# google/dynibar

Hardware: AMD Instinct MI355X
Metric: rays/sec (64 samples x 8 src views) (higher is better)
Workload: dtype f32 in / f32 accumulate; products from two half-float parts per operand (22-bit operands, 3 of the 4 partial products on the f16 matrix pipe, ~2^-20 relative per product); the exact 6-term bf16 build is tested beside it

## Files before the change

dynibar_amd/build.py:

```python
from __future__ import annotations

import os
import subprocess
import sys

HERE = os.path.dirname(os.path.abspath(__file__))
CSRC = os.path.join(HERE, 'csrc')
OUT = os.path.join(CSRC, 'libdynibar_hip.so')
OUT_X6 = os.path.join(CSRC, 'libdynibar_hip_x6.so')
OUT_X1 = os.path.join(CSRC, 'libdynibar_hip_x1.so')
UNITS = [
    ('dyn_geometry.hip', ['-ffp-contract=off', '-munsafe-fp-atomics']),
    ('dyn_nets.hip', []),
    ('dyn_encoder.hip', ['-munsafe-fp-atomics']),
    ('dyn_train.hip', ['-munsafe-fp-atomics']),
    ('dyn_comm.hip', []),
]
COMMON = ['--offload-arch=gfx950', '-O3', '-std=c++17', '-fPIC', '-Wall', '-Wno-unused-function']
FLAVOURS = [
    ('dyn_nets_x6.o', OUT_X6, ['-DDYN_SPLIT_TERMS=6', '-DDYN_SPLIT_F16=0']),
    ('dyn_nets_x1.o', OUT_X1, ['-DDYN_SPLIT_TERMS=1']),
]


def _deps():
  return [os.path.join(CSRC, f) for f in os.listdir(CSRC) if f.endswith(('.hip', '.h'))] + [
      os.path.join(os.path.dirname(HERE), 'include', 'dynibar_hip.h')]


STAMP = os.path.join(CSRC, '.build_stamp')


def _stamp():
  import hashlib
  h = hashlib.sha256(repr((COMMON, UNITS, [(o, os.path.basename(out), f) for o, out, f in FLAVOURS])).encode())
  for d in sorted(_deps() + [os.path.abspath(__file__)]):
    h.update(os.path.basename(d).encode())
    with open(d, 'rb') as f:
      h.update(f.read())
  return h.hexdigest()


def build(force=False, verbose=True):
  hipcc = os.environ.get('HIPCC', '/opt/rocm/bin/hipcc')
  units = [(s, f) for s, f in UNITS if os.path.exists(os.path.join(CSRC, s))]
  stamp = _stamp()
  if not force and all(os.path.exists(p) for p in [OUT, STAMP] + [out for _, out, _ in FLAVOURS]) and open(STAMP).read().strip() == stamp:
    return OUT
  if os.path.exists(STAMP):
    os.remove(STAMP)
  from concurrent.futures import ThreadPoolExecutor
  jobs = []
  for src, flags in units:
    obj = os.path.join(CSRC, src.replace('.hip', '.o'))
    jobs.append((obj, [hipcc] + COMMON + flags + ['-c', os.path.join(CSRC, src), '-o', obj]))
  for obj, _, flags in FLAVOURS:
    jobs.append((os.path.join(CSRC, obj), [hipcc] + COMMON + flags + ['-c', os.path.join(CSRC, 'dyn_nets.hip'), '-o', os.path.join(CSRC, obj)]))

  def run(job):
    if verbose:
      print(' '.join(job[1]), flush=True)
    subprocess.check_call(job[1])
    return job[0]

  with ThreadPoolExecutor(max_workers=int(os.environ.get('DYNIBAR_BUILD_JOBS', '6'))) as ex:
    built = list(ex.map(run, jobs))
  objs = built[:len(units)]
  cmd = [hipcc, '--offload-arch=gfx950', '-shared', '-fPIC'] + objs + ['-ldl', '-o', OUT]
  if verbose:
    print(' '.join(cmd), flush=True)
  subprocess.check_call(cmd)
  for flavour, (_, out, _) in zip(built[len(units):], FLAVOURS):
    subprocess.check_call([hipcc, '--offload-arch=gfx950', '-shared', '-fPIC', objs[0], flavour] + objs[2:] + ['-ldl', '-o', out])
  if _stamp() == stamp:
    with open(STAMP, 'w') as f:
      f.write(stamp + '\n')
  return OUT


if __name__ == '__main__':
  print(build(force='--force' in sys.argv))
```

dynibar_amd/csrc/dyn_mlp.h:

```cpp
#pragma once
#include <utility>

#include "dyn_device.h"

#ifndef DYN_EXCLUSIVE_CU
#define DYN_EXCLUSIVE_CU 1
#endif
#if DYN_EXCLUSIVE_CU && defined(__AMDGCN__)
#define DYN_CLAIM_REGISTER_FILE() asm volatile("; the whole register file" ::: "v255", "a255")
#else
#define DYN_CLAIM_REGISTER_FILE()
#endif
#define DYN_NET_THREADS 256
#define DYN_VIEW_THREADS 512

__host__ __device__ constexpr int dyn_fi(int r, int h) { return (r & 3) + 8 * (r >> 2) + 4 * h; }

__device__ __forceinline__ f32x16 mfma32(float a, float b, f32x16 c) { return __builtin_amdgcn_mfma_f32_32x32x2f32(a, b, c, 0, 0, 0); }

template <int NT>
__device__ __forceinline__ void acc_zero(f32x16 (&acc)[NT]) {
#pragma unroll
  for (int t = 0; t < NT; ++t)
#pragma unroll
// ... 105 lines not shown
  a = seg_sum<VSEG>(a, 0, 0); b = seg_sum<VSEG>(b, 0, 0); c = seg_sum<VSEG>(c, 0, 0); d = seg_sum<VSEG>(d, 0, 0);
}
template <int VSEG>
__device__ __forceinline__ float seg_min(float v, int, int) {
  return seg_reduce<VSEG>(v, [](float a, float b) { return fminf(a, b); });
}
template <int VSEG>
__device__ __forceinline__ float seg_max(float v, int, int) {
  return seg_reduce<VSEG>(v, [](float a, float b) { return fmaxf(a, b); });
}

template <int NTI>
__device__ __forceinline__ float row_dot(const f32x16 (&act)[NTI], const float* tab) {
  const int h = (threadIdx.x & 63) >> 5;
  const float4* t4 = reinterpret_cast<const float4*>(tab + h * 16 * NTI);
  float s = 0.f;
#pragma unroll
  for (int t = 0; t < NTI; ++t)
#pragma unroll
    for (int q = 0; q < 4; ++q) {
      const float4 w = t4[t * 4 + q];
      s = fmaf(act[t][q * 4 + 0], w.x, s);
      s = fmaf(act[t][q * 4 + 1], w.y, s);
      s = fmaf(act[t][q * 4 + 2], w.z, s);
      s = fmaf(act[t][q * 4 + 3], w.w, s);
    }
  return s + __shfl_xor(s, 32);
}

#ifndef DYN_SPLIT_TERMS
#define DYN_SPLIT_TERMS 3
#endif
#ifndef DYN_SPLIT_F16
#define DYN_SPLIT_F16 1
#endif
#if DYN_SPLIT_F16 && DYN_SPLIT_TERMS == 6
#error "the half-float engine has one or two parts per operand (DYN_SPLIT_TERMS == 1 or 3)"
#endif
#if !DYN_SPLIT_F16 && DYN_SPLIT_TERMS == 1
#error "the one-product engine multiplies IEEE halves (DYN_SPLIT_F16 == 1)"
#endif
#if DYN_SPLIT_TERMS == 1
#define DYN_SPLIT_PARTS 1
#define B6_CHUNK_PAIRS 48
#elif DYN_SPLIT_TERMS == 3
#define DYN_SPLIT_PARTS 2
#define B6_CHUNK_PAIRS 24
#elif DYN_SPLIT_TERMS == 6
#define DYN_SPLIT_PARTS 3
#define B6_CHUNK_PAIRS 16
#else
#error "DYN_SPLIT_TERMS must be 1, 3 or 6"
#endif
#define DYN_BIAS_ONE(h) ((DYN_SPLIT_TERMS == 1 || (h) == 0) ? 1.0f : 0.0f)
typedef __bf16 bf16x8 __attribute__((ext_vector_type(8)));
typedef __bf16 bf16x2v __attribute__((ext_vector_type(2)));
typedef _Float16 f16x8 __attribute__((ext_vector_type(8)));
typedef _Float16 f16x2v __attribute__((ext_vector_type(2)));
typedef float f32x2v __attribute__((ext_vector_type(2)));
typedef unsigned u32x4v __attribute__((ext_vector_type(4)));

#define B6_PAIR_FLOATS (DYN_SPLIT_PARTS * 256)
#define B6_CHUNK (B6_CHUNK_PAIRS * B6_PAIR_FLOATS)

#ifdef DYN_PHASE_TIMING
__device__ unsigned long long g_phase[3][2][160];
#define DYN_PHASE_ON (threadIdx.x == 0 && (blockIdx.x == 0 || blockIdx.x == gridDim.x / 2))
#define DYN_PHASE(i)                                                                                  \
  do {                                                                                                \
    if (DYN_PHASE_ON) g_phase[PHASE_KID][blockIdx.x != 0][i] = __builtin_readcyclecounter();          \
  } while (0)
extern "C" int dyn_debug_phases(unsigned long long* out) {
  return hipMemcpyFromSymbol(out, HIP_SYMBOL(g_phase), sizeof(g_phase)) == hipSuccess ? 0 : 1;
}
#define DYN_PHASE_T0 const unsigned long long phase_t0 = __builtin_readcyclecounter();
#ifdef DYN_PHASE_SKEW
__device__ unsigned long long g_skew[8][4];
extern "C" int dyn_debug_skew(unsigned long long* out) { return hipMemcpyFromSymbol(out, HIP_SYMBOL(g_skew), sizeof(g_skew)) == hipSuccess ? 0 : 1; }
extern "C" int dyn_debug_skew_reset(void) { unsigned long long z[32] = {0}; return hipMemcpyToSymbol(HIP_SYMBOL(g_skew), z, sizeof(z)) == hipSuccess ? 0 : 1; }
#endif
#define DYN_PHASE_WAIT(R, c)                                                                          \
  do {                                                                                                \
    if (DYN_PHASE_ON && (c) < 64) {                                                                   \
      g_phase[(R).kid][blockIdx.x != 0][32 + (c)] = __builtin_readcyclecounter() - phase_t0;          \
      g_phase[(R).kid][blockIdx.x != 0][96 + (c)] = phase_t0;                                         \
    }                                                                                                 \
  } while (0)
#define DYN_PHASE_RING_KID(R, k) (R).kid = (k)
#else
#define DYN_PHASE(i)
#define DYN_PHASE_T0
#define DYN_PHASE_WAIT(R, c)
#define DYN_PHASE_RING_KID(R, k)
#endif

struct WeightRing6 {
  const float* gbase;
  float* buf;
  int next, total;
  int skip_at, skip_n;
  int round;
  int half;
  unsigned lds_wave;
  unsigned lane_off;
  int fill, issued;
  int nbuf;
// ... 192 lines not shown
#if DYN_SPLIT_PARTS == 3
  f32x2v mf = {__uint_as_float(mid << 16), __uint_as_float(mid & 0xffff0000u)};
  f32x2v r2 = r1 - mf;
  lo = __builtin_bit_cast(unsigned, __builtin_convertvector(r2, bf16x2v));
#else
  lo = 0u;
#endif
#endif
}

__device__ __forceinline__ f32x16 mfma_bf16(u32x4v a, u32x4v b, f32x16 c) {
#if DYN_SPLIT_F16
  return __builtin_amdgcn_mfma_f32_32x32x16_f16(__builtin_bit_cast(f16x8, a), __builtin_bit_cast(f16x8, b), c, 0, 0, 0);
#else
  return __builtin_amdgcn_mfma_f32_32x32x16_bf16(__builtin_bit_cast(bf16x8, a), __builtin_bit_cast(bf16x8, b), c, 0, 0, 0);
#endif
}

__host__ __device__ constexpr int b6_layer_chunks(int NT, int NSLOTS, int CP = B6_CHUNK_PAIRS) {
  return (((NSLOTS + 7) / 8) + (CP / NT) - 1) / (CP / NT);
}

struct B6A {
  u32x4v hi, mid, lo;
};
__device__ __forceinline__ B6A b6_load_a(const float* pair, int lane) {
  const u32x4v* w = reinterpret_cast<const u32x4v*>(pair) + lane;
  B6A a;
  a.hi = w[0];
#if DYN_SPLIT_PARTS >= 2
  a.mid = w[64];
#endif
#if DYN_SPLIT_PARTS == 3
  a.lo = w[128];
#endif
  return a;
}

template <int NSLOTS, int P0, int P1, class Feed>
__device__ __forceinline__ void b6_split_pairs(Feed& feed, int g, u32x4v& bh, u32x4v& bm, u32x4v& bl) {
#pragma unroll
  for (int p2 = P0; p2 < P1; ++p2) {
    const float v0 = (g * 8 + 2 * p2 < NSLOTS) ? feed(g * 8 + 2 * p2) : 0.f;
    const float v1 = (g * 8 + 2 * p2 + 1 < NSLOTS) ? feed(g * 8 + 2 * p2 + 1) : 0.f;
    unsigned h_, m_, l_;
    split3_pair(v0, v1, h_, m_, l_);
    bh[p2] = h_; bm[p2] = m_; bl[p2] = l_;
  }
}

#ifndef B6_AHEAD
#define B6_AHEAD 1
#endif
template <int NT, int NSLOTS, int AHEAD = B6_AHEAD, class Feed>
__device__ __forceinline__ void mlp_layer_b6(WeightRing6& R, f32x16 (&acc)[NT], Feed&& feed) {
  constexpr int NG = (NSLOTS + 7) / 8;
  constexpr int GPC = B6_CHUNK_PAIRS / NT;
  constexpr int NCH = (NG + GPC - 1) / GPC;
  static_assert(B6_CHUNK_PAIRS % NT == 0, "tiles per layer must divide the pairs of a chunk");
  static_assert(NT == 1 || NT == 2 || NT == 4 || NT == 8, "output tiles per layer");
  const int lane = threadIdx.x & 63;
  u32x4v bh, bm, bl, nh, nm, nl;
  b6_split_pairs<NSLOTS, 0, 4>(feed, 0, bh, bm, bl);
  nh = bh; nm = bm; nl = bl;
  __builtin_amdgcn_sched_barrier(0);
#pragma unroll
  for (int c = 0; c < NCH; ++c) {
    const float* buf = ring6_acquire(R);
    constexpr int NPC_MAX = B6_CHUNK_PAIRS;
    const int npc = (NG - c * GPC < GPC ? NG - c * GPC : GPC) * NT;
    B6A q[AHEAD + 1];
#pragma unroll
    for (int i = 0; i < AHEAD; ++i)
      if (i < npc) q[i] = b6_load_a(buf + i * B6_PAIR_FLOATS, lane);
    __builtin_amdgcn_sched_barrier(0);
#pragma unroll
    for (int pr = 0; pr < NPC_MAX; ++pr) {
      if (pr < npc) {
        const int gi = pr / NT, t = pr % NT;
        const int g = c * GPC + gi;
        ring6_feed(R, pr, npc);
#if B6_PRIO_FLIP && (B6_PRIO_MODE == 1 || B6_PRIO_MODE == 5)
        if (pr % B6_PRIO_FLIP == 0) ring6_prio_flip(R, (pr / B6_PRIO_FLIP) & 1);
#endif
        if (pr + AHEAD < npc) q[(pr + AHEAD) % (AHEAD + 1)] = b6_load_a(buf + (pr + AHEAD) * B6_PAIR_FLOATS, lane);
        if (g + 1 < NG) {
          if (NT == 1) b6_split_pairs<NSLOTS, 0, 4>(feed, g + 1, nh, nm, nl);
          if (NT == 2 && t == 0) b6_split_pairs<NSLOTS, 0, 2>(feed, g + 1, nh, nm, nl);
          if (NT == 2 && t == 1) b6_split_pairs<NSLOTS, 2, 4>(feed, g + 1, nh, nm, nl);
          if (NT == 4 && t == 0) b6_split_pairs<NSLOTS, 0, 1>(feed, g + 1, nh, nm, nl);
          if (NT == 4 && t == 1) b6_split_pairs<NSLOTS, 1, 2>(feed, g + 1, nh, nm, nl);
          if (NT == 4 && t == 2) b6_split_pairs<NSLOTS, 2, 3>(feed, g + 1, nh, nm, nl);
          if (NT == 4 && t == 3) b6_split_pairs<NSLOTS, 3, 4>(feed, g + 1, nh, nm, nl);
          if (NT == 8 && t == 0) b6_split_pairs<NSLOTS, 0, 1>(feed, g + 1, nh, nm, nl);
          if (NT == 8 && t == 2) b6_split_pairs<NSLOTS, 1, 2>(feed, g + 1, nh, nm, nl);
          if (NT == 8 && t == 4) b6_split_pairs<NSLOTS, 2, 3>(feed, g + 1, nh, nm, nl);
          if (NT == 8 && t == 6) b6_split_pairs<NSLOTS, 3, 4>(feed, g + 1, nh, nm, nl);
        }
        const B6A& cur = q[pr % (AHEAD + 1)];
#if DYN_SPLIT_TERMS == 6
        acc[t] = mfma_bf16(cur.lo, bh, acc[t]);
        acc[t] = mfma_bf16(cur.hi, bl, acc[t]);
        acc[t] = mfma_bf16(cur.mid, bm, acc[t]);
#endif
#if DYN_SPLIT_TERMS != 1
        acc[t] = mfma_bf16(cur.mid, bh, acc[t]);
        acc[t] = mfma_bf16(cur.hi, bm, acc[t]);
#endif
        acc[t] = mfma_bf16(cur.hi, bh, acc[t]);
        if (t == NT - 1) { bh = nh; bm = nm; bl = nl; }
        __builtin_amdgcn_sched_barrier(0);
      }
    }
  }
}

#ifndef B6D_AHEAD
#define B6D_AHEAD 4
#endif
#define B6D_SLOTS 3
struct WeightRing3 {
  const float* gbase;
  const float* glane;
  float* buf;
  unsigned lds_wave;
  unsigned lane_off;
  int next, total;
  int waves;
  int cf;
  int fill, issued;
  float* slot[B6D_SLOTS];
  unsigned lds_slot[B6D_SLOTS];
#ifdef DYN_PHASE_TIMING
  int kid;
#endif
};
template <int OFF>
__device__ __forceinline__ void ring3_dma(const float* g, float* l_emu, unsigned l, const float* g_uniform, unsigned lane_off) {
#if defined(__AMDGCN__)
#pragma clang diagnostic push
#pragma clang diagnostic ignored "-Winline-asm"
  asm volatile("s_mov_b32 m0, %2\n\ts_nop 0\n\tglobal_load_lds_dwordx4 %0, %1 offset:%3" ::"v"(lane_off), "s"(g_uniform), "s"(l), "n"(OFF) : "m0", "memory");
#pragma clang diagnostic pop
#else
  __builtin_amdgcn_global_load_lds((const __attribute__((address_space(1))) void*)g, (__attribute__((address_space(3))) void*)l_emu, 16, OFF, 0);
#endif
}
__device__ __forceinline__ int ring3_pieces(const WeightRing3& R) { return R.cf / (R.waves * 256); }
__device__ __forceinline__ void ring3_piece(const WeightRing3& R, int chunk, int k) {
  const int per_wave = R.cf / R.waves;
  const int grp = k / 6, i = k % 6;
  const float* g = R.glane + (long)chunk * R.cf + grp * 1536;
  const float* gu = R.gbase + (long)chunk * R.cf + grp * 1536;
  const unsigned l = R.lds_slot[chunk % B6D_SLOTS] + (unsigned)(grp * 1536 * sizeof(float));
  float* le = R.slot[chunk % B6D_SLOTS] + (threadIdx.x >> 6) * per_wave + 512 + grp * 1536;
  if (i == 0) ring3_dma<-2048>(g, le, l, gu, R.lane_off);
  if (i == 1) ring3_dma<-1024>(g, le, l, gu, R.lane_off);
  if (i == 2) ring3_dma<0>(g, le, l, gu, R.lane_off);
  if (i == 3) ring3_dma<1024>(g, le, l, gu, R.lane_off);
  if (i == 4) ring3_dma<2048>(g, le, l, gu, R.lane_off);
  if (i == 5) ring3_dma<3072>(g, le, l, gu, R.lane_off);
}
template <int ALLOW = 0>
__device__ __forceinline__ void ring3_barrier() {
#if defined(__AMDGCN__)
  static_assert(ALLOW >= 0 && ALLOW < 16, "vmcnt immediate");
  __builtin_amdgcn_s_waitcnt(0x0F70 | ALLOW);
// ... 206 lines not shown
    };
    auto dma = [&](auto D) DYN_INLINE_LAMBDA {
      constexpr int done = decltype(D)::value;
      constexpr int wend = mid - B6D_DMA_MARGIN;
      if constexpr (pr >= mid) ring3_feed(R, 0, pr + done - mid, npc - mid);
      else if constexpr (wend <= 0) ring3_feed(R, 1, 1, 1);
      else ring3_feed(R, 1, pr + done < wend ? pr + done : wend, wend);
    };
    if constexpr (P + AHEAD < NP) q[(P + AHEAD) % QN] = load(P + AHEAD);
    gap(std::integral_constant<int, 0>{});
    const B6A& a0 = q[P % QN];
    const B6A& a1 = q[(P + U - 1) % QN];
#if DYN_SPLIT_TERMS == 6
    acc[t0] = mfma_pinned<ACC_AGPR>(a0.lo, bh, acc[t0]);
    if constexpr (U == 2) acc[t1] = mfma_pinned<ACC_AGPR>(a1.lo, bh, acc[t1]);
    acc[t0] = mfma_pinned<ACC_AGPR>(a0.hi, bl, acc[t0]);
    if constexpr (U == 2) acc[t1] = mfma_pinned<ACC_AGPR>(a1.hi, bl, acc[t1]);
    acc[t0] = mfma_pinned<ACC_AGPR>(a0.mid, bm, acc[t0]);
    if constexpr (U == 2) acc[t1] = mfma_pinned<ACC_AGPR>(a1.mid, bm, acc[t1]);
#endif
    if constexpr (DYN_SPLIT_TERMS != 1) acc[t0] = mfma_pinned<ACC_AGPR>(a0.mid, bh, acc[t0]);
    __builtin_amdgcn_sched_barrier(0);
    if constexpr (U == 2) {
      if constexpr (P + AHEAD + 1 < NP) q[(P + AHEAD + 1) % QN] = load(P + AHEAD + 1);
      gap(std::integral_constant<int, 1>{});
      if constexpr (DYN_SPLIT_TERMS != 1) acc[t1] = mfma_pinned<ACC_AGPR>(a1.mid, bh, acc[t1]);
      __builtin_amdgcn_sched_barrier(0);
      gap(std::integral_constant<int, 2>{});
    }
    if constexpr (DYN_SPLIT_TERMS != 1) acc[t0] = mfma_pinned<ACC_AGPR>(a0.hi, bm, acc[t0]);
    if constexpr (U == 2) {
      __builtin_amdgcn_sched_barrier(0);
      gap(std::integral_constant<int, 3>{});
      dma(std::integral_constant<int, 1>{});
      if constexpr (DYN_SPLIT_TERMS != 1) acc[t1] = mfma_pinned<ACC_AGPR>(a1.hi, bm, acc[t1]);
      __builtin_amdgcn_sched_barrier(0);
      gap(std::integral_constant<int, 4>{});
    }
    acc[t0] = mfma_pinned<ACC_AGPR>(a0.hi, bh, acc[t0]);
    if constexpr (U == 2) {
      __builtin_amdgcn_sched_barrier(0);
      gap(std::integral_constant<int, 5>{});
      dma(std::integral_constant<int, U>{});
      acc[t1] = mfma_pinned<ACC_AGPR>(a1.hi, bh, acc[t1]);
    } else {
      dma(std::integral_constant<int, U>{});
    }
    if constexpr (t1 == NT - 1) { bh = nh; bm = nm; bl = nl; }
    if constexpr (pr + U == npc) ring3_leave(R);
    __builtin_amdgcn_sched_barrier(0);
  });
}

template <int NT, int NSLOTS, int AHEAD = B6_AHEAD, class Feed>
__device__ __forceinline__ void mlp_layer_b6_lds(const float* w, f32x16 (&acc)[NT], Feed&& feed) {
  constexpr int NG = (NSLOTS + 7) / 8, NPR = NG * NT;
  static_assert(NT == 1 || NT == 2 || NT == 4 || NT == 8, "output tiles per layer");
  const int lane = threadIdx.x & 63;
  u32x4v bh, bm, bl, nh, nm, nl;
  b6_split_pairs<NSLOTS, 0, 4>(feed, 0, bh, bm, bl);
  nh = bh; nm = bm; nl = bl;
  B6A q[AHEAD + 1];
#pragma unroll
  for (int i = 0; i < AHEAD; ++i)
    if (i < NPR) q[i] = b6_load_a(w + i * B6_PAIR_FLOATS, lane);
  __builtin_amdgcn_sched_barrier(0);
#pragma unroll
  for (int pr = 0; pr < NPR; ++pr) {
    const int g = pr / NT, t = pr % NT;
    if (pr + AHEAD < NPR) q[(pr + AHEAD) % (AHEAD + 1)] = b6_load_a(w + (pr + AHEAD) * B6_PAIR_FLOATS, lane);
    if (g + 1 < NG) {
      if (NT == 1) b6_split_pairs<NSLOTS, 0, 4>(feed, g + 1, nh, nm, nl);
      if (NT == 2 && t == 0) b6_split_pairs<NSLOTS, 0, 2>(feed, g + 1, nh, nm, nl);
      if (NT == 2 && t == 1) b6_split_pairs<NSLOTS, 2, 4>(feed, g + 1, nh, nm, nl);
      if (NT == 4 && t == 0) b6_split_pairs<NSLOTS, 0, 1>(feed, g + 1, nh, nm, nl);
      if (NT == 4 && t == 1) b6_split_pairs<NSLOTS, 1, 2>(feed, g + 1, nh, nm, nl);
      if (NT == 4 && t == 2) b6_split_pairs<NSLOTS, 2, 3>(feed, g + 1, nh, nm, nl);
      if (NT == 4 && t == 3) b6_split_pairs<NSLOTS, 3, 4>(feed, g + 1, nh, nm, nl);
      if (NT == 8 && t == 0) b6_split_pairs<NSLOTS, 0, 1>(feed, g + 1, nh, nm, nl);
      if (NT == 8 && t == 2) b6_split_pairs<NSLOTS, 1, 2>(feed, g + 1, nh, nm, nl);
      if (NT == 8 && t == 4) b6_split_pairs<NSLOTS, 2, 3>(feed, g + 1, nh, nm, nl);
      if (NT == 8 && t == 6) b6_split_pairs<NSLOTS, 3, 4>(feed, g + 1, nh, nm, nl);
    }
    const B6A& cur = q[pr % (AHEAD + 1)];
#if DYN_SPLIT_TERMS == 6
    acc[t] = mfma_bf16(cur.lo, bh, acc[t]);
    acc[t] = mfma_bf16(cur.hi, bl, acc[t]);
    acc[t] = mfma_bf16(cur.mid, bm, acc[t]);
#endif
#if DYN_SPLIT_TERMS != 1
    acc[t] = mfma_bf16(cur.mid, bh, acc[t]);
    acc[t] = mfma_bf16(cur.hi, bm, acc[t]);
#endif
    acc[t] = mfma_bf16(cur.hi, bh, acc[t]);
    if (t == NT - 1) { bh = nh; bm = nm; bl = nl; }
    __builtin_amdgcn_sched_barrier(0);
  }
}

template <int NSLOTS>
struct B6TileW {
  B6A a[(NSLOTS + 7) / 8];
};
template <int NT, int NSLOTS>
__device__ __forceinline__ void b6_tile_prefetch(const float* layer_chunks, int my_tile, B6TileW<NSLOTS>& w) {
  constexpr int NG = (NSLOTS + 7) / 8;
  constexpr int GPC = B6_CHUNK_PAIRS / NT;
  const int lane = threadIdx.x & 63;
#pragma unroll
  for (int g = 0; g < NG; ++g) w.a[g] = b6_load_a(layer_chunks + (g / GPC) * B6_CHUNK + ((g % GPC) * NT + my_tile) * B6_PAIR_FLOATS, lane);
}
template <int NSLOTS, class Feed>
__device__ __forceinline__ void b6_tile_apply(const B6TileW<NSLOTS>& w, f32x16& acc, Feed&& feed) {
  constexpr int NG = (NSLOTS + 7) / 8;
#pragma unroll
  for (int g = 0; g < NG; ++g) {
    u32x4v bh, bm, bl;
    b6_split_pairs<NSLOTS, 0, 4>(feed, g, bh, bm, bl);
#if DYN_SPLIT_TERMS == 6
    acc = mfma_bf16(w.a[g].lo, bh, acc);
    acc = mfma_bf16(w.a[g].hi, bl, acc);
    acc = mfma_bf16(w.a[g].mid, bm, acc);
#endif
#if DYN_SPLIT_TERMS != 1
    acc = mfma_bf16(w.a[g].mid, bh, acc);
    acc = mfma_bf16(w.a[g].hi, bm, acc);
#endif
    acc = mfma_bf16(w.a[g].hi, bh, acc);
  }
}

typedef WeightRing6 NetRing;
#define NET_CHUNK B6_CHUNK
#define net_ring_init ring6_init
#define net_ring_init_t(R, stream, total, lds, threads) ring6_init(R, stream, total, lds, 1 << 30, 0, threads)
#define net_ring_init_1(R, stream, total, lds, threads) ring6_init(R, stream, total, lds, 1 << 30, 0, threads, 1)
#define net_layer mlp_layer_b6
__host__ __device__ constexpr int net_layer_chunks(int NT, int NSLOTS) { return b6_layer_chunks(NT, NSLOTS); }
```

dynibar_amd/csrc/dyn_nets.hip:

```cpp
#include <math.h>
#include <stdlib.h>
#include <string.h>

#include <functional>
#include <vector>

#include "dyn_host.h"
#include "dyn_mlp.h"
#include "dyn_pack.h"

namespace {

using SlotFn = std::function<float(int t, int i, int s, int h)>;

thread_local bool g_pack_slot_error = false;
thread_local int g_pack_chunk_pairs = B6_CHUNK_PAIRS;
void pack_layer_b6(std::vector<float>& out, int NT, int NSLOTS, const SlotFn& fn, int ones_slot = -1) {
  const int CPAIRS = g_pack_chunk_pairs, CFLOATS = CPAIRS * B6_PAIR_FLOATS;
  const int NG = (NSLOTS + 7) / 8, GPC = CPAIRS / NT, NCH = (NG + GPC - 1) / GPC;
  const size_t base = out.size();
  out.resize(base + (size_t)NCH * CFLOATS, 0.f);
  unsigned short* img = reinterpret_cast<unsigned short*>(out.data() + base);
  for (int c = 0; c < NCH; ++c)
    for (int gi = 0; gi < GPC; ++gi) {
// ... 877 lines not shown
}

template <int VSEG, bool STORE_X>
__device__ __forceinline__ void views_tail(NetRing& ring, f32x16 (&a1)[8], const StaticArgs& p, const float* ctab, float wgt, float msk,
                                           long tile, long point, bool valid, int view, int seg_base, const DenseRows* dr = nullptr,
                                           float* lds_base = nullptr, int v_const = 0) {
  constexpr int PHASE_KID = 0;
  (void)PHASE_KID;
  const int lane = threadIdx.x & 63, h = lane >> 5;
  const int V = v_const > 0 ? v_const : p.V;
  f32x16 x[4];
  {
    acc_init_bias<4>(x, ctab + 272);
    net_layer<4, SA_L4_STEPS>(ring, x, [&](int s) { return elu_s(a1[s / 16][s % 16]); });
    DYN_PHASE(11);
  }
  float vis;
  {
    f32x16 a5[4], a6[4];
    acc_init_bias<4>(a5, ctab + 400);
    DYN_PHASE(12);
    net_layer<4, SA_L5_STEPS>(ring, a5, [&](int s) {
      const float r = elu1(x[s / 16][s % 16]);
      x[s / 16][s % 16] = r;
      return r * wgt;
    });
    DYN_PHASE(13);
    acc_init_bias<4>(a6, ctab + 528);
    net_layer<4, SA_L5_STEPS>(ring, a6, [&](int s) {
      const float r = elu_s(a5[s / 16][s % 16]);
      a5[s / 16][s % 16] = r;
      return r;
    });
    DYN_PHASE(14);
    vis = sigmoid1(elu1(row_dot<4>(a5, ctab) + ctab[256])) * msk;
#pragma unroll
    for (int t = 0; t < 4; ++t)
#pragma unroll
      for (int r = 0; r < 16; ++r) x[t][r] += elu1(a6[t][r]);
  }
  float vis2;
  {
    f32x16 a7[4];
    acc_init_bias<4>(a7, ctab + 656);
    DYN_PHASE(15);
    net_layer<4, SA_L5_STEPS>(ring, a7, [&](int s) { return x[s / 16][s % 16] * vis; });
    DYN_PHASE(16);
    acc_elu_s(a7);
    vis2 = sigmoid1(row_dot<4>(a7, ctab + 128) + ctab[257]) * msk;
  }
  DYN_PHASE(17);
  const bool tile_ok = tile < p.n_tiles_a;
  if (STORE_X && tile_ok) {
    float4* xw = reinterpret_cast<float4*>(p.ws + p.o.off_x) + tile * 16 * 64 + lane;
#pragma unroll
    for (int t = 0; t < 4; ++t)
#pragma unroll
      for (int q = 0; q < 4; ++q) nt_store4<4>(xw + (t * 4 + q) * 64, make_float4(x[t][q * 4], x[t][q * 4 + 1], x[t][q * 4 + 2], x[t][q * 4 + 3]));
    if (h == 0) nt_store1<4>(p.ws + p.o.off_vis + (tile * 32 + (lane & 31)) * 4, vis2);
  }
  DYN_PHASE(18);
  if constexpr (VSEG == 0) {
    const DenseRows& d = *dr;
    const int tid = threadIdx.x;
    float vsum, nvalid;
    dense_all2(d, vis2, msk, vsum, nvalid);
    const float w2 = vis2 / (vsum + 1e-8f);
    const float wmean = (vsum / (vsum + 1e-8f)) / (float)V;
    constexpr int XS = 132;
    float* tab = lds_base;
    float* wrow = lds_base + 256 * XS;
    const long point0 = d.point0;
    {
      float4* mine = reinterpret_cast<float4*>(tab + d.rw * XS) + h;
#pragma unroll
      for (int t = 0; t < 4; ++t)
#pragma unroll
        for (int q = 0; q < 4; ++q) mine[8 * t + 2 * q] = make_float4(x[t][q * 4], x[t][q * 4 + 1], x[t][q * 4 + 2], x[t][q * 4 + 3]);
      if (h == 0) wrow[d.rw] = w2;
    }
    __syncthreads();
    for (int task = tid; task < d.PTW * 32; task += DYN_VIEW_THREADS) {
      const int pnt = task >> 5, qd = task & 31;
      const int pb = dense_pt_base(d, pnt), pn = dense_pt_cnt(d, pnt);
      const float* src = tab + pb * XS + qd * 4;
      const float* w = wrow + pb;
      float4 m0 = make_float4(0.f, 0.f, 0.f, 0.f), m1 = m0;
      int k = 0;
      for (; k + 2 <= pn; k += 2) {
        const float4 x0 = dense_quad(src, k, XS, pn), x1 = dense_quad(src, k + 1, XS, pn);
        const float w0 = dense_w(w, k, pn), w1 = dense_w(w, k + 1, pn);
        m0.x = fmaf(w0, x0.x, m0.x); m0.y = fmaf(w0, x0.y, m0.y); m0.z = fmaf(w0, x0.z, m0.z); m0.w = fmaf(w0, x0.w, m0.w);
        m1.x = fmaf(w1, x1.x, m1.x); m1.y = fmaf(w1, x1.y, m1.y); m1.z = fmaf(w1, x1.z, m1.z); m1.w = fmaf(w1, x1.w, m1.w);
      }
      if (k < pn) {
        const float4 x0 = dense_quad(src, k, XS, pn);
        const float w0 = dense_w(w, k, pn);
        m0.x = fmaf(w0, x0.x, m0.x); m0.y = fmaf(w0, x0.y, m0.y); m0.z = fmaf(w0, x0.z, m0.z); m0.w = fmaf(w0, x0.w, m0.w);
      }
      const float mean[4] = {m0.x + m1.x, m0.y + m1.y, m0.z + m1.z, m0.w + m1.w};
      float v0[4] = {0.f, 0.f, 0.f, 0.f}, v1[4] = {0.f, 0.f, 0.f, 0.f};
      for (k = 0; k + 2 <= pn; k += 2) {
        const float4 x0 = dense_quad(src, k, XS, pn), x1 = dense_quad(src, k + 1, XS, pn);
        const float w0 = dense_w(w, k, pn), w1 = dense_w(w, k + 1, pn);
        const float a0[4] = {x0.x, x0.y, x0.z, x0.w}, b0[4] = {x1.x, x1.y, x1.z, x1.w};
#pragma unroll
        for (int e = 0; e < 4; ++e) {
          const float d0 = a0[e] - mean[e], d1 = b0[e] - mean[e];
          v0[e] = fmaf(w0, d0 * d0, v0[e]);
          v1[e] = fmaf(w1, d1 * d1, v1[e]);
        }
// ... 889 lines not shown
      f32x16 a8[8];
      acc_zero(a8);
      PTS8_LAYER(8, 64)(ring, a8, [&](int s) { return g[s / 16][s % 16]; });
      float pe[17];
      float c3[3] = {0.f, 0.f, 0.f};
      if (valid) { c3[0] = p.pts[point * 3]; c3[1] = p.pts[point * 3 + 1]; c3[2] = p.pts[point * 3 + 2]; }
#pragma unroll
      for (int c = 0; c < 3; ++c) octave_embed<5>(c3[c], h_t, pe + c * 5);
      pe[15] = h_t == 0 ? c3[0] : c3[1];
      pe[16] = h_t == 0 ? c3[2] : 1.0f;
      PTS8_LAYER(8, 17)(ring, a8, [&](int s) { return pe[s]; });
      acc_zero(g2);
      PTS8_LAYER(4, 129)(ring, g2, [&](int s) { return s < 128 ? elu_s(a8[s / 16][s % 16]) : one_h0_t; });
    }
    f32x16 a[4];
    acc_zero(a);
    PTS8_LAYER(4, 65)(ring, a, [&](int s) {
      if (s >= 64) return one_h0_t;
      const float r = elu1(g2[s / 16][s % 16]);
      g2[s / 16][s % 16] = r;
      return r;
    });
    acc_elu_s(a);
    float sigma = row_dot<4>(a, ctab + 256) + ctab[384] - p.shift;
    if (few_views) sigma = -1e9f;
    float pd[14];
    {
      float d3[3] = {0.f, 0.f, 1.f};
      if (valid) unit3(p.ray_d[ray * 3], p.ray_d[ray * 3 + 1], p.ray_d[ray * 3 + 2], d3[0], d3[1], d3[2]);
#pragma unroll
      for (int c = 0; c < 3; ++c) octave_embed<4>(d3[c], h_t, pd + c * 4);
      pd[12] = h_t == 0 ? d3[0] : d3[1];
      pd[13] = h_t == 0 ? d3[2] : 1.0f;
    }
    acc_zero(a);
    PTS8_LAYER(4, 78)(ring, a, [&](int s) { return s < 64 ? g2[s / 16][s % 16] : pd[s - 64]; });
    f32x16 b2[2];
    acc_zero(b2);
    PTS8_LAYER(2, 65)(ring, b2, [&](int s) { return s < 64 ? elu_s(a[s / 16][s % 16]) : one_h0_t; });
    acc_elu_s(b2);
    float rgb[3];
#pragma unroll
    for (int c = 0; c < 3; ++c) {
      rgb[c] = sigmoid1(row_dot<2>(b2, ctab + 400 + c * 64) + ctab[385 + c]);
      if (no_view) rgb[c] = 0.f;
    }
    if (valid && h_t == 0) reinterpret_cast<float4*>(p.raw)[point] = make_float4(rgb[0], rgb[1], rgb[2], sigma);
  }
  DYN_PHASE(20);
}
#endif

#define DYN_BLEND_THREADS 256
template <int VSEG, int THREADS>
__device__ __forceinline__ void static_blend_body(StaticArgs p) {
  constexpr int PHASE_KID = 2;
  (void)PHASE_KID;
  DYN_PHASE(0);
  float* lds = reinterpret_cast<float*>(dyn_smem);
  float* ctab = lds + NET_CHUNK;
  const int tid = threadIdx.x, lane = tid & 63, j = lane & 31, h = lane >> 5, wave = tid >> 6;
  for (int i = tid; i < SC_CT; i += THREADS) ctab[i] = p.blob[ST_OFF_CTC + i];
  NetRing ring;
  net_ring_init_1(ring, p.blob + ST_OFF_C, SC_CHUNKS, lds, THREADS);
  DYN_PHASE_RING_KID(ring, 2);

  const int V = p.V;
  const long tile = (long)blockIdx.x * (THREADS / 64) + wave;
  const bool tile_ok = tile < p.n_tiles_a;
  const DenseRows dr = dense_rows(V, p.PT, ctab + SC_CT);
  const int p_local = VSEG == 0 ? dr.p_local : j / (VSEG == 0 ? 1 : VSEG);
  const int view = VSEG == 0 ? dr.view : (j & (VSEG - 1));
  const long point = VSEG == 0 ? (long)blockIdx.x * p.PT + p_local : tile * p.PT + p_local;
  const bool valid = (VSEG == 0 ? p_local < p.PT : view < V) && (point < p.n_pts);
  const long pv = valid ? point * V + view : 0;

  float msk = valid ? p.mask[pv] : 0.f;
  const float4 rd = valid ? reinterpret_cast<const float4*>(p.ray_diff)[pv] : make_float4(0.f, 0.f, 0.f, 0.f);
  const float4 vrec = tile_ok ? reinterpret_cast<const float4*>(p.ws + p.o.off_vis)[tile * 32 + j] : make_float4(0.f, 0.f, 0.f, 0.f);
  const float vis2 = vrec.x;
  const float rgb_in[3] = {valid ? vrec.y : 0.f, valid ? vrec.z : 0.f, valid ? vrec.w : 0.f};
  if (p.mask_rgb && !((rgb_in[0] + rgb_in[1]) + rgb_in[2] > 1e-3f)) msk = 0.f;
  f32x16 a[4];
  {
    f32x16 x[4];
    const float4* xw = reinterpret_cast<const float4*>(p.ws + p.o.off_x) + (tile_ok ? tile : 0) * 16 * 64 + lane;
    const float4* hg = reinterpret_cast<const float4*>(p.ws + p.o.off_hg) + (valid ? point_rec(p, point, h, SB_HG_RECS) : 0);
#pragma unroll
    for (int t = 0; t < 4; ++t)
#pragma unroll
      for (int q = 0; q < 4; ++q) {
        const float4 v = tile_ok ? nt_load4<8>(xw + (t * 4 + q) * 64) : make_float4(0.f, 0.f, 0.f, 0.f);
        x[t][q * 4] = v.x; x[t][q * 4 + 1] = v.y; x[t][q * 4 + 2] = v.z; x[t][q * 4 + 3] = v.w;
        const float4 b = valid ? hg[(t * 4 + q) * 64] : make_float4(0.f, 0.f, 0.f, 0.f);
        a[t][q * 4] = b.x; a[t][q * 4 + 1] = b.y; a[t][q * 4 + 2] = b.z; a[t][q * 4 + 3] = b.w;
      }
    const float extra[3] = {h == 0 ? vis2 : rd.x, h == 0 ? rd.y : rd.z, h == 0 ? rd.w : 0.f};
    net_layer<4, SC_L11_STEPS>(ring, a, [&](int s) { return s < 64 ? x[s / 16][s % 16] : extra[s - 64]; });
  }
  f32x16 b2[2];
  acc_init_bias<2>(b2, ctab + 80);
  net_layer<2, 64>(ring, b2, [&](int s) { return elu_s(a[s / 16][s % 16]); });
  acc_elu_s(b2);
  float logit = row_dot<2>(b2, ctab) + ctab[64];
  if (msk == 0.f) logit = -1e9f;
  if (VSEG == 0 ? p_local >= p.PT : view >= V) logit = -3.0e38f;
  const float mx = views_max<VSEG>(dr, logit);
  const float e = (VSEG == 0 && p_local >= p.PT) ? 0.f : __expf(logit - mx);
  const float bw = e / views_sum<VSEG>(dr, e);
#pragma unroll
  for (int c = 0; c < 3; ++c) {
    const float v = views_sum<VSEG>(dr, rgb_in[c] * bw);
    if (valid && (VSEG == 0 ? dr.rw == dr.base : view == 0) && h == 0) p.raw[point * 4 + c] = v;
  }
  DYN_PHASE(20);
}
#define SC_L11_PAIRS (((SC_L11_STEPS + 7) / 8) * 4)
#define SC_L12_PAIRS ((64 / 8) * 2)
#define SC_WS_FLOATS ((SC_L11_PAIRS + SC_L12_PAIRS) * B6_PAIR_FLOATS)
#ifndef DYN_BLEND_WS_THREADS
#define DYN_BLEND_WS_THREADS 512
#endif
#if DYN_BLEND_WS
__device__ __forceinline__ long n_units_of(const StaticArgs& p, bool rag, int vseg, int nw) {
  return rag ? p.rg_wg[0] : (vseg == 0 ? (p.n_tiles_a + nw - 1) / nw : p.n_tiles_a);
}
template <int VSEG, int THREADS, bool RAG = false>
__device__ __forceinline__ void static_blend_ws_body(StaticArgs p) {
  float* lds = reinterpret_cast<float*>(dyn_smem);
  float* ctab = lds + SC_WS_FLOATS;
  const int tid = threadIdx.x, lane = tid & 63, j = lane & 31, h = lane >> 5, wave = tid >> 6;
  for (int i = tid; i < SC_CT; i += THREADS) ctab[i] = p.blob[ST_OFF_CTC + i];
  {
    constexpr int CP = B6_CHUNK_PAIRS, L11_CH = net_layer_chunks(4, SC_L11_STEPS);
    const float4* src = reinterpret_cast<const float4*>(p.blob + ST_OFF_C);
    float4* dst = reinterpret_cast<float4*>(lds);
    for (int i = tid; i < SC_WS_FLOATS / 4; i += THREADS) {
      const int pair = i / (B6_PAIR_FLOATS / 4), within = i - pair * (B6_PAIR_FLOATS / 4);
      const int sp = pair < SC_L11_PAIRS ? pair : L11_CH * CP + (pair - SC_L11_PAIRS);
      dst[i] = src[(long)sp * (B6_PAIR_FLOATS / 4) + within];
    }
  }
  __syncthreads();
  const float* w11 = lds;
  const float* w12 = lds + SC_L11_PAIRS * B6_PAIR_FLOATS;
  const int V = p.V;
  constexpr int NW = THREADS / 64;
  DenseRows dr = dense_rows(V, p.PT, ctab + SC_CT, 0);
#ifndef DYN_BLEND_PREFETCH
#define DYN_BLEND_PREFETCH 1
#endif
  f32x16 x[4];
  auto tile_of = [&](long u_) { return VSEG == 0 ? u_ * NW + wave : u_; };
  auto load_x = [&](long u_, int t) DYN_INLINE_LAMBDA {
    const long tl = tile_of(u_);
    const bool ok = u_ < n_units_of(p, RAG, VSEG, NW) && tl < p.n_tiles_a;
    const float4* xw = reinterpret_cast<const float4*>(p.ws + p.o.off_x) + (ok ? tl : 0) * 16 * 64 + lane;
#pragma unroll
    for (int q = 0; q < 4; ++q) {
      const float4 v = ok ? nt_load4<8>(xw + (t * 4 + q) * 64) : make_float4(0.f, 0.f, 0.f, 0.f);
      x[t][q * 4] = v.x; x[t][q * 4 + 1] = v.y; x[t][q * 4 + 2] = v.z; x[t][q * 4 + 3] = v.w;
    }
  };
  const long n_units = n_units_of(p, RAG, VSEG, NW);
  const long first = VSEG == 0 ? blockIdx.x : (long)blockIdx.x * NW + wave, step = VSEG == 0 ? gridDim.x : (long)gridDim.x * NW;
  if (DYN_BLEND_PREFETCH) {
#pragma unroll
    for (int t = 0; t < 4; ++t) load_x(first, t);
  }
  RaggedHead head_next = {0, 0, 0, 0};
  if (RAG && first < n_units) head_next = ragged_head(p.rg_rowtab, p.rg_ptab, first, dr.rw);
  for (long u = first; u < n_units; u += step) {
    if (RAG) {
      const RaggedHead head = head_next;
      if (u + step < n_units) head_next = ragged_head(p.rg_rowtab, p.rg_ptab, u + step, dr.rw);
      dr = ragged_rows(V, p.rg_rowtab, p.rg_ptab, u, ctab + SC_CT, nullptr, &head);
    } else if (VSEG == 0) {
      dr.point0 = u * p.PT;
    }
    const int PT = RAG ? dr.PTW : p.PT;
    const int p_local = VSEG == 0 ? dr.p_local : j / (VSEG == 0 ? 1 : VSEG);
    const int view = VSEG == 0 ? dr.view : (j & (VSEG - 1));
    const long tile = VSEG == 0 ? u * NW + wave : u;
    const bool tile_ok = tile < p.n_tiles_a;
    const long point = VSEG == 0 ? dr.point0 + p_local : tile * PT + p_local;
    const bool valid = (VSEG == 0 ? p_local < PT : view < V) && (point < p.n_pts);
    const long pv = valid ? point * V + view : 0;
    float msk = valid ? p.mask[pv] : 0.f;
    const float4 rd = valid ? reinterpret_cast<const float4*>(p.ray_diff)[pv] : make_float4(0.f, 0.f, 0.f, 0.f);
    const float4 vrec = tile_ok ? reinterpret_cast<const float4*>(p.ws + p.o.off_vis)[tile * 32 + j] : make_float4(0.f, 0.f, 0.f, 0.f);
    const float vis2 = vrec.x;
    const float rgb_in[3] = {valid ? vrec.y : 0.f, valid ? vrec.z : 0.f, valid ? vrec.w : 0.f};
    if (p.mask_rgb && !((rgb_in[0] + rgb_in[1]) + rgb_in[2] > 1e-3f)) msk = 0.f;
    f32x16 a[4];
    {
      const float4* hg = reinterpret_cast<const float4*>(p.ws + p.o.off_hg) + (valid ? point_rec(p, point, h, SB_HG_RECS) : 0);
#pragma unroll
      for (int t = 0; t < 4; ++t) {
        if (!DYN_BLEND_PREFETCH) load_x(u, t);
#pragma unroll
        for (int q = 0; q < 4; ++q) {
          const float4 b = valid ? hg[(t * 4 + q) * 64] : make_float4(0.f, 0.f, 0.f, 0.f);
          a[t][q * 4] = b.x; a[t][q * 4 + 1] = b.y; a[t][q * 4 + 2] = b.z; a[t][q * 4 + 3] = b.w;
        }
      }
      const float extra[3] = {h == 0 ? vis2 : rd.x, h == 0 ? rd.y : rd.z, h == 0 ? rd.w : 0.f};
      mlp_layer_b6_lds<4, SC_L11_STEPS>(w11, a, [&](int s) { return s < 64 ? x[s / 16][s % 16] : extra[s - 64]; });
    }
    f32x16 b2[2];
    acc_init_bias<2>(b2, ctab + 80);
    mlp_layer_b6_lds<2, 64>(w12, b2, [&](int s) {
      const float r = elu_s(a[s / 16][s % 16]);
      if (DYN_BLEND_PREFETCH && (s & 15) == 15) load_x(u + step, s / 16);
      return r;
    });
    acc_elu_s(b2);
    float logit = row_dot<2>(b2, ctab) + ctab[64];
    if (msk == 0.f) logit = -1e9f;
    if (VSEG == 0 ? p_local >= PT : view >= V) logit = -3.0e38f;
    const float mx = views_max<VSEG>(dr, logit);
    const float e = (VSEG == 0 && p_local >= PT) ? 0.f : __expf(logit - mx);
    const float bw = e / views_sum<VSEG>(dr, e);
    const bool writer = valid && (VSEG == 0 ? dr.rw == dr.base : view == 0) && h == 0;
    const bool all_masked = RAG && writer && p.ws[p.o.off_nvalid + point] == 0.f;
#pragma unroll
    for (int c = 0; c < 3; ++c) {
      float v = views_sum<VSEG>(dr, rgb_in[c] * bw);
      if (all_masked) {
        const float wv = 1.0f / (float)V;
        v = 0.f;
        for (int k = 0; k < V; ++k) v += p.rgb_feat[(point * V + k) * 35 + c] * wv;
      }
      if (writer) p.raw[point * 4 + c] = v;
    }
  }
}
template <int VSEG>
__global__ void __launch_bounds__(DYN_BLEND_WS_THREADS, 1) k_static_blend_ws(StaticArgs p) { static_blend_ws_body<VSEG, DYN_BLEND_WS_THREADS>(p); }
template <bool RAG>
__global__ void __launch_bounds__(DYN_VIEW_THREADS, 1) k_static_blend_dense_ws(StaticArgs p) { static_blend_ws_body<0, DYN_VIEW_THREADS, RAG>(p); }
#endif

template <int VSEG>
__global__ void __launch_bounds__(DYN_BLEND_THREADS, 3) k_static_blend(StaticArgs p) { static_blend_body<VSEG, DYN_BLEND_THREADS>(p); }
__global__ void __launch_bounds__(DYN_VIEW_THREADS, 1) k_static_blend_dense(StaticArgs p) { static_blend_body<0, DYN_VIEW_THREADS>(p); }


static int ragged_plan(StaticArgs& a, const float* s_abs, hipStream_t stream) {
  unsigned* bits = reinterpret_cast<unsigned*>(a.ws + a.o.off_bits);
  float* emin = a.ws + a.o.off_emin;
  int* seg_cnt = reinterpret_cast<int*>(a.ws + a.o.off_segcnt);
  int* seg_start = reinterpret_cast<int*>(a.ws + a.o.off_segstart);
  int* wg = reinterpret_cast<int*>(a.ws + a.o.off_wgstart);
  unsigned short* rowtab = reinterpret_cast<unsigned short*>(a.ws + a.o.off_rowtab);
  int* ptab = reinterpret_cast<int*>(a.ws + a.o.off_ptab);
  a.rg_bits = bits; a.rg_emin = emin; a.rg_wg = wg; a.rg_rowtab = rowtab; a.rg_ptab = ptab;
  DYN_REQUIRE(a.n_pts < (1L << 31), "ragged plan: R * S must stay below 2^31 points");
  DYN_LAUNCH(DYN_K_STATIC_PLAN, "k_ragged_points", k_ragged_points, dim3(dyn_cdiv(a.n_pts, 256)), dim3(256), (size_t)256 * a.V * 5, stream, a.n_pts, a.V, a.mask,
             reinterpret_cast<const float4*>(a.ray_diff), s_abs, bits, emin);
  DYN_LAUNCH(DYN_K_STATIC_PLAN, "k_ragged_segments", k_ragged_segments, dim3((unsigned)a.o.n_seg), dim3(256), (RAG_SEG + 4 + 256) * sizeof(int) + RAG_SEG * sizeof(unsigned short), stream, a.n_pts, a.o.n_seg, bits, seg_cnt, seg_start);
// ... 537 lines not shown
```

Measured before the change: 1.551 million.

## Park pre-split half-float parts of x instead of f32 for blend layer

The producer kernel that stores the x features now stores them already split into the half-float hi/mid packed parts. The blend kernels load these parts and feed them straight into the matrix ops through a new 'ready operand' hook, skipping the per-use split for the first 8 groups. This removes repeated split arithmetic in the blend inner loop at the cost of a different workspace layout and a split in the producer. With two parts per operand the number of stored quads stays at four per tile. A separate f32-parked build flavour is kept for comparison.

Result: no change. 1.548 million (-0.2%).

```diff
diff --git a/dynibar_amd/build.py b/dynibar_amd/build.py
--- a/dynibar_amd/build.py
+++ b/dynibar_amd/build.py
@@ -9,6 +9,7 @@
 OUT = os.path.join(CSRC, 'libdynibar_hip.so')
 OUT_X6 = os.path.join(CSRC, 'libdynibar_hip_x6.so')
 OUT_X1 = os.path.join(CSRC, 'libdynibar_hip_x1.so')
+OUT_PARK_F32 = os.path.join(CSRC, 'libdynibar_hip_parkf32.so')
 UNITS = [
     ('dyn_geometry.hip', ['-ffp-contract=off', '-munsafe-fp-atomics']),
     ('dyn_nets.hip', []),
@@ -20,6 +21,7 @@
 FLAVOURS = [
     ('dyn_nets_x6.o', OUT_X6, ['-DDYN_SPLIT_TERMS=6', '-DDYN_SPLIT_F16=0']),
     ('dyn_nets_x1.o', OUT_X1, ['-DDYN_SPLIT_TERMS=1']),
+    ('dyn_nets_parkf32.o', OUT_PARK_F32, ['-DDYN_PARK_X_SPLIT=0']),
 ]
 
 
@@ -63,7 +65,7 @@
     subprocess.check_call(job[1])
     return job[0]
 
-  with ThreadPoolExecutor(max_workers=int(os.environ.get('DYNIBAR_BUILD_JOBS', '6'))) as ex:
+  with ThreadPoolExecutor(max_workers=int(os.environ.get('DYNIBAR_BUILD_JOBS', '8'))) as ex:
     built = list(ex.map(run, jobs))
   objs = built[:len(units)]
   cmd = [hipcc, '--offload-arch=gfx950', '-shared', '-fPIC'] + objs + ['-ldl', '-o', OUT]
diff --git a/dynibar_amd/csrc/dyn_mlp.h b/dynibar_amd/csrc/dyn_mlp.h
--- a/dynibar_amd/csrc/dyn_mlp.h
+++ b/dynibar_amd/csrc/dyn_mlp.h
@@ -181,6 +181,13 @@
 #else
 #error "DYN_SPLIT_TERMS must be 1, 3 or 6"
 #endif
+#ifndef DYN_PARK_X_SPLIT
+#define DYN_PARK_X_SPLIT (DYN_SPLIT_PARTS <= 2 ? 1 : 0)
+#endif
+#if DYN_PARK_X_SPLIT && DYN_SPLIT_PARTS == 3
+#error "DYN_PARK_X_SPLIT needs an engine with one or two parts per operand"
+#endif
+#define DYN_PARK_X_QUADS (DYN_PARK_X_SPLIT ? 2 * DYN_SPLIT_PARTS : 4)
 #define DYN_BIAS_ONE(h) ((DYN_SPLIT_TERMS == 1 || (h) == 0) ? 1.0f : 0.0f)
 typedef __bf16 bf16x8 __attribute__((ext_vector_type(8)));
 typedef __bf16 bf16x2v __attribute__((ext_vector_type(2)));
@@ -479,17 +486,23 @@
 #ifndef B6_AHEAD
 #define B6_AHEAD 1
 #endif
-template <int NT, int NSLOTS, int AHEAD = B6_AHEAD, class Feed>
-__device__ __forceinline__ void mlp_layer_b6(WeightRing6& R, f32x16 (&acc)[NT], Feed&& feed) {
+struct B6NoReady {
+  __device__ __forceinline__ void operator()(int, u32x4v&, u32x4v&) const {}
+};
+template <int NT, int NSLOTS, int NREADY, int AHEAD = B6_AHEAD, class Feed, class Ready>
+__device__ __forceinline__ void mlp_layer_b6_pre(WeightRing6& R, f32x16 (&acc)[NT], Feed&& feed, Ready&& ready) {
   constexpr int NG = (NSLOTS + 7) / 8;
   constexpr int GPC = B6_CHUNK_PAIRS / NT;
   constexpr int NCH = (NG + GPC - 1) / GPC;
   static_assert(B6_CHUNK_PAIRS % NT == 0, "tiles per layer must divide the pairs of a chunk");
   static_assert(NT == 1 || NT == 2 || NT == 4 || NT == 8, "output tiles per layer");
+  static_assert(NREADY == 0 || (DYN_SPLIT_PARTS <= 2 && NREADY <= NG), "ready operands have one or two parts");
   const int lane = threadIdx.x & 63;
   u32x4v bh, bm, bl, nh, nm, nl;
-  b6_split_pairs<NSLOTS, 0, 4>(feed, 0, bh, bm, bl);
-  nh = bh; nm = bm; nl = bl;
+  if constexpr (NREADY == 0) {
+    b6_split_pairs<NSLOTS, 0, 4>(feed, 0, bh, bm, bl);
+    nh = bh; nm = bm; nl = bl;
+  }
   __builtin_amdgcn_sched_barrier(0);
 #pragma unroll
   for (int c = 0; c < NCH; ++c) {
@@ -511,7 +524,7 @@
         if (pr % B6_PRIO_FLIP == 0) ring6_prio_flip(R, (pr / B6_PRIO_FLIP) & 1);
 #endif
         if (pr + AHEAD < npc) q[(pr + AHEAD) % (AHEAD + 1)] = b6_load_a(buf + (pr + AHEAD) * B6_PAIR_FLOATS, lane);
-        if (g + 1 < NG) {
+        if (g + 1 < NG && g + 1 >= NREADY) {
           if (NT == 1) b6_split_pairs<NSLOTS, 0, 4>(feed, g + 1, nh, nm, nl);
           if (NT == 2 && t == 0) b6_split_pairs<NSLOTS, 0, 2>(feed, g + 1, nh, nm, nl);
           if (NT == 2 && t == 1) b6_split_pairs<NSLOTS, 2, 4>(feed, g + 1, nh, nm, nl);
@@ -525,6 +538,9 @@
           if (NT == 8 && t == 6) b6_split_pairs<NSLOTS, 3, 4>(feed, g + 1, nh, nm, nl);
         }
         const B6A& cur = q[pr % (AHEAD + 1)];
+        if constexpr (NREADY > 0) {
+          if (g < NREADY) ready(g, bh, bm);
+        }
 #if DYN_SPLIT_TERMS == 6
         acc[t] = mfma_bf16(cur.lo, bh, acc[t]);
         acc[t] = mfma_bf16(cur.hi, bl, acc[t]);
@@ -535,11 +551,15 @@
         acc[t] = mfma_bf16(cur.hi, bm, acc[t]);
 #endif
         acc[t] = mfma_bf16(cur.hi, bh, acc[t]);
-        if (t == NT - 1) { bh = nh; bm = nm; bl = nl; }
+        if (t == NT - 1 && g + 1 >= NREADY) { bh = nh; bm = nm; bl = nl; }
         __builtin_amdgcn_sched_barrier(0);
       }
     }
   }
+}
+template <int NT, int NSLOTS, int AHEAD = B6_AHEAD, class Feed>
+__device__ __forceinline__ void mlp_layer_b6(WeightRing6& R, f32x16 (&acc)[NT], Feed&& feed) {
+  mlp_layer_b6_pre<NT, NSLOTS, 0, AHEAD>(R, acc, feed, B6NoReady{});
 }
 
 #ifndef B6D_AHEAD
@@ -852,14 +872,17 @@
   });
 }
 
-template <int NT, int NSLOTS, int AHEAD = B6_AHEAD, class Feed>
-__device__ __forceinline__ void mlp_layer_b6_lds(const float* w, f32x16 (&acc)[NT], Feed&& feed) {
+template <int NT, int NSLOTS, int NREADY, int AHEAD = B6_AHEAD, class Feed, class Ready>
+__device__ __forceinline__ void mlp_layer_b6_lds_pre(const float* w, f32x16 (&acc)[NT], Feed&& feed, Ready&& ready) {
   constexpr int NG = (NSLOTS + 7) / 8, NPR = NG * NT;
   static_assert(NT == 1 || NT == 2 || NT == 4 || NT == 8, "output tiles per layer");
+  static_assert(NREADY == 0 || (DYN_SPLIT_PARTS <= 2 && NREADY <= NG), "ready operands have one or two parts");
   const int lane = threadIdx.x & 63;
   u32x4v bh, bm, bl, nh, nm, nl;
-  b6_split_pairs<NSLOTS, 0, 4>(feed, 0, bh, bm, bl);
-  nh = bh; nm = bm; nl = bl;
+  if constexpr (NREADY == 0) {
+    b6_split_pairs<NSLOTS, 0, 4>(feed, 0, bh, bm, bl);
+    nh = bh; nm = bm; nl = bl;
+  }
   B6A q[AHEAD + 1];
 #pragma unroll
   for (int i = 0; i < AHEAD; ++i)
@@ -869,7 +892,7 @@
   for (int pr = 0; pr < NPR; ++pr) {
     const int g = pr / NT, t = pr % NT;
     if (pr + AHEAD < NPR) q[(pr + AHEAD) % (AHEAD + 1)] = b6_load_a(w + (pr + AHEAD) * B6_PAIR_FLOATS, lane);
-    if (g + 1 < NG) {
+    if (g + 1 < NG && g + 1 >= NREADY) {
       if (NT == 1) b6_split_pairs<NSLOTS, 0, 4>(feed, g + 1, nh, nm, nl);
       if (NT == 2 && t == 0) b6_split_pairs<NSLOTS, 0, 2>(feed, g + 1, nh, nm, nl);
       if (NT == 2 && t == 1) b6_split_pairs<NSLOTS, 2, 4>(feed, g + 1, nh, nm, nl);
@@ -883,6 +906,9 @@
       if (NT == 8 && t == 6) b6_split_pairs<NSLOTS, 3, 4>(feed, g + 1, nh, nm, nl);
     }
     const B6A& cur = q[pr % (AHEAD + 1)];
+    if constexpr (NREADY > 0) {
+      if (g < NREADY) ready(g, bh, bm);
+    }
 #if DYN_SPLIT_TERMS == 6
     acc[t] = mfma_bf16(cur.lo, bh, acc[t]);
     acc[t] = mfma_bf16(cur.hi, bl, acc[t]);
@@ -893,9 +919,13 @@
     acc[t] = mfma_bf16(cur.hi, bm, acc[t]);
 #endif
     acc[t] = mfma_bf16(cur.hi, bh, acc[t]);
-    if (t == NT - 1) { bh = nh; bm = nm; bl = nl; }
+    if (t == NT - 1 && g + 1 >= NREADY) { bh = nh; bm = nm; bl = nl; }
     __builtin_amdgcn_sched_barrier(0);
   }
+}
+template <int NT, int NSLOTS, int AHEAD = B6_AHEAD, class Feed>
+__device__ __forceinline__ void mlp_layer_b6_lds(const float* w, f32x16 (&acc)[NT], Feed&& feed) {
+  mlp_layer_b6_lds_pre<NT, NSLOTS, 0, AHEAD>(w, acc, feed, B6NoReady{});
 }
 
 template <int NSLOTS>
diff --git a/dynibar_amd/csrc/dyn_nets.hip b/dynibar_amd/csrc/dyn_nets.hip
--- a/dynibar_amd/csrc/dyn_nets.hip
+++ b/dynibar_amd/csrc/dyn_nets.hip
@@ -953,11 +953,29 @@
   DYN_PHASE(17);
   const bool tile_ok = tile < p.n_tiles_a;
   if (STORE_X && tile_ok) {
-    float4* xw = reinterpret_cast<float4*>(p.ws + p.o.off_x) + tile * 16 * 64 + lane;
+    float4* xw = reinterpret_cast<float4*>(p.ws + p.o.off_x) + tile * (4 * DYN_PARK_X_QUADS) * 64 + lane;
+#if DYN_PARK_X_SPLIT
 #pragma unroll
     for (int t = 0; t < 4; ++t)
 #pragma unroll
+      for (int gg = 0; gg < 2; ++gg) {
+        u32x4v bh, bm;
+#pragma unroll
+        for (int p2 = 0; p2 < 4; ++p2) {
+          unsigned h_, m_, l_;
+          split3_pair(x[t][gg * 8 + 2 * p2], x[t][gg * 8 + 2 * p2 + 1], h_, m_, l_);
+          bh[p2] = h_; bm[p2] = m_;
+        }
+        float4* xg = xw + (t * 2 + gg) * DYN_SPLIT_PARTS * 64;
+        nt_store4<4>(xg, make_float4(__uint_as_float(bh[0]), __uint_as_float(bh[1]), __uint_as_float(bh[2]), __uint_as_float(bh[3])));
+        if (DYN_SPLIT_PARTS == 2) nt_store4<4>(xg + 64, make_float4(__uint_as_float(bm[0]), __uint_as_float(bm[1]), __uint_as_float(bm[2]), __uint_as_float(bm[3])));
+      }
+#else
+#pragma unroll
+    for (int t = 0; t < 4; ++t)
+#pragma unroll
       for (int q = 0; q < 4; ++q) nt_store4<4>(xw + (t * 4 + q) * 64, make_float4(x[t][q * 4], x[t][q * 4 + 1], x[t][q * 4 + 2], x[t][q * 4 + 3]));
+#endif
     if (h == 0) nt_store1<4>(p.ws + p.o.off_vis + (tile * 32 + (lane & 31)) * 4, vis2);
   }
   DYN_PHASE(18);
@@ -1953,6 +1971,19 @@
 #endif
 
 #define DYN_BLEND_THREADS 256
+struct BlendX {
+  dyn_f32x4 q[4][DYN_PARK_X_QUADS];
+  __device__ __forceinline__ void set(int t, int i, float4 v) { q[t][i] = dyn_f32x4{v.x, v.y, v.z, v.w}; }
+  __device__ __forceinline__ float slot(int s) const { return q[s / 16][(s % 16) / 4][s % 4]; }
+  __device__ __forceinline__ void operator()(int g, u32x4v& hi, u32x4v& mid) const {
+#if DYN_PARK_X_SPLIT
+    hi = __builtin_bit_cast(u32x4v, q[g / 2][(g % 2) * DYN_SPLIT_PARTS]);
+#if DYN_SPLIT_PARTS == 2
+    mid = __builtin_bit_cast(u32x4v, q[g / 2][(g % 2) * 2 + 1]);
+#endif
+#endif
+  }
+};
 template <int VSEG, int THREADS>
 __device__ __forceinline__ void static_blend_body(StaticArgs p) {
   constexpr int PHASE_KID = 2;
@@ -1984,20 +2015,25 @@
   if (p.mask_rgb && !((rgb_in[0] + rgb_in[1]) + rgb_in[2] > 1e-3f)) msk = 0.f;
   f32x16 a[4];
   {
-    f32x16 x[4];
-    const float4* xw = reinterpret_cast<const float4*>(p.ws + p.o.off_x) + (tile_ok ? tile : 0) * 16 * 64 + lane;
+    BlendX x;
+    const float4* xw = reinterpret_cast<const float4*>(p.ws + p.o.off_x) + (tile_ok ? tile : 0) * (4 * DYN_PARK_X_QUADS) * 64 + lane;
     const float4* hg = reinterpret_cast<const float4*>(p.ws + p.o.off_hg) + (valid ? point_rec(p, point, h, SB_HG_RECS) : 0);
 #pragma unroll
-    for (int t = 0; t < 4; ++t)
+    for (int t = 0; t < 4; ++t) {
+#pragma unroll
+      for (int q = 0; q < DYN_PARK_X_QUADS; ++q) x.set(t, q, tile_ok ? nt_load4<8>(xw + (t * DYN_PARK_X_QUADS + q) * 64) : make_float4(0.f, 0.f, 0.f, 0.f));
 #pragma unroll
       for (int q = 0; q < 4; ++q) {
-        const float4 v = tile_ok ? nt_load4<8>(xw + (t * 4 + q) * 64) : make_float4(0.f, 0.f, 0.f, 0.f);
-        x[t][q * 4] = v.x; x[t][q * 4 + 1] = v.y; x[t][q * 4 + 2] = v.z; x[t][q * 4 + 3] = v.w;
         const float4 b = valid ? hg[(t * 4 + q) * 64] : make_float4(0.f, 0.f, 0.f, 0.f);
         a[t][q * 4] = b.x; a[t][q * 4 + 1] = b.y; a[t][q * 4 + 2] = b.z; a[t][q * 4 + 3] = b.w;
       }
+    }
     const float extra[3] = {h == 0 ? vis2 : rd.x, h == 0 ? rd.y : rd.z, h == 0 ? rd.w : 0.f};
-    net_layer<4, SC_L11_STEPS>(ring, a, [&](int s) { return s < 64 ? x[s / 16][s % 16] : extra[s - 64]; });
+#if DYN_PARK_X_SPLIT
+    mlp_layer_b6_pre<4, SC_L11_STEPS, 8>(ring, a, [&](int s) { return extra[s - 64]; }, x);
+#else
+    net_layer<4, SC_L11_STEPS>(ring, a, [&](int s) { return s < 64 ? x.slot(s) : extra[s - 64]; });
+#endif
   }
   f32x16 b2[2];
   acc_init_bias<2>(b2, ctab + 80);
@@ -2051,17 +2087,14 @@
 #ifndef DYN_BLEND_PREFETCH
 #define DYN_BLEND_PREFETCH 1
 #endif
-  f32x16 x[4];
+  BlendX x;
   auto tile_of = [&](long u_) { return VSEG == 0 ? u_ * NW + wave : u_; };
   auto load_x = [&](long u_, int t) DYN_INLINE_LAMBDA {
     const long tl = tile_of(u_);
     const bool ok = u_ < n_units_of(p, RAG, VSEG, NW) && tl < p.n_tiles_a;
-    const float4* xw = reinterpret_cast<const float4*>(p.ws + p.o.off_x) + (ok ? tl : 0) * 16 * 64 + lane;
-#pragma unroll
-    for (int q = 0; q < 4; ++q) {
-      const float4 v = ok ? nt_load4<8>(xw + (t * 4 + q) * 64) : make_float4(0.f, 0.f, 0.f, 0.f);
-      x[t][q * 4] = v.x; x[t][q * 4 + 1] = v.y; x[t][q * 4 + 2] = v.z; x[t][q * 4 + 3] = v.w;
-    }
+    const float4* xw = reinterpret_cast<const float4*>(p.ws + p.o.off_x) + (ok ? tl : 0) * (4 * DYN_PARK_X_QUADS) * 64 + lane;
+#pragma unroll
+    for (int q = 0; q < DYN_PARK_X_QUADS; ++q) x.set(t, q, ok ? nt_load4<8>(xw + (t * DYN_PARK_X_QUADS + q) * 64) : make_float4(0.f, 0.f, 0.f, 0.f));
   };
   const long n_units = n_units_of(p, RAG, VSEG, NW);
   const long first = VSEG == 0 ? blockIdx.x : (long)blockIdx.x * NW + wave, step = VSEG == 0 ? gridDim.x : (long)gridDim.x * NW;
@@ -2106,7 +2139,11 @@
         }
       }
       const float extra[3] = {h == 0 ? vis2 : rd.x, h == 0 ? rd.y : rd.z, h == 0 ? rd.w : 0.f};
-      mlp_layer_b6_lds<4, SC_L11_STEPS>(w11, a, [&](int s) { return s < 64 ? x[s / 16][s % 16] : extra[s - 64]; });
+#if DYN_PARK_X_SPLIT
+      mlp_layer_b6_lds_pre<4, SC_L11_STEPS, 8>(w11, a, [&](int s) { return extra[s - 64]; }, x);
+#else
+      mlp_layer_b6_lds<4, SC_L11_STEPS>(w11, a, [&](int s) { return s < 64 ? x.slot(s) : extra[s - 64]; });
+#endif
     }
     f32x16 b2[2];
     acc_init_bias<2>(b2, ctab + 80);
```
